# GEM3D/pressurePoissonSolver

Hardware: AMD Instinct MI355X
Metric: V-cycle lattice-site updates/sec, 512^3 3D Poisson (higher is better)
Workload: dtype f64; 1 GPU; apps/3d/steady-equivalent: 512^3 uniform, 4096 patches of 32^3, 5 levels, V(1,1), smoother=rbgs, Dirichlet, f ~ U(-1,1) splitmix64(0x5EED + patch id); workload_key=3d:u512:p32:rbgs, parallelism=patch-sharded x1 (Morton ranges), exchange=none, levels=5, smoother=rbgs

## Files before the change

### pressurepoissonsolver_amd/csrc/dispatch.hpp

```cpp
#pragma once
#include <cstddef>
#include <type_traits>

namespace tei
{
template <class F> inline auto dispatchN(int n, F f)
{
	switch (n) {
		case 4: return f(std::integral_constant<int, 4>{});
		case 8: return f(std::integral_constant<int, 8>{});
		case 16: return f(std::integral_constant<int, 16>{});
		default: return f(std::integral_constant<int, 32>{});
	}
}

template <class F> inline auto dispatchBool(bool b, F f)
{
	return b ? f(std::true_type{}) : f(std::false_type{});
}

template <int N, class F> inline void dispatchSlabs(int slabs, F f)
{
	switch (slabs) {
		case 1: f(std::integral_constant<int, 1>{}); break;
		case 2:
// ... 29 lines not shown
	}
	return zs;
}

inline int rbgsSlabCount(int n, int count, const SlabSwitches &s)
{
	if (s.pin) return pinnedSlabs(n, s.pin);
	int zs = 1;
	while (zs < 4 && !s.rbgs_noslab && (size_t) count * zs < 1024 && n / (zs * 2) >= 4) zs *= 2;
	if (zs == 4 && n == 32 && count <= 64 && !s.no_zs8) zs = 8;
	return zs;
}

constexpr size_t kResweepCacheBytes = (size_t) 160 << 20;

inline bool resweepPinValid(int pin) { return pin == 19 || pin == 27 || pin == 59; }

inline int resweepVariant(bool exported_terms, bool refined, int index, size_t level_bytes, int pin)
{
	if (exported_terms) return refined ? 0 : 3;
	const int v = pin ? pin : (index != 0 ? 27 : (level_bytes <= kResweepCacheBytes ? 19 : 59));
	return (refined && v == 19) ? 27 : v;
}
}
```

### pressurepoissonsolver_amd/csrc/gmg_core.hip

```cpp
#include "gmg_internal.hpp"

namespace tei
{
const char *kclassName[KC_COUNT] = {"stencil_apply", "stencil_resid", "stencil_jacobi", "stencil_rbgs",
                                    "cf_ghost", "restrict", "prolong_add", "patch_rhs", "dst_axis",
                                    "vecop", "reduce", "pack", "exchange", "stencil_rbgs_zero", "resid_restrict", "patch_solve_mfma", "stencil_rbgs_prolong",
                                    "stencil_rbgs_slabs", "stencil_slabs", "patch_solve_3pass", "rbgs_zero_resid_restrict",
                                    "restrict_fixup", "rbgs_resweep_prolong", "rbgs_zero_resid_restrict_faces",
                                    "rbgs_resweep_prolong_fcorr", "rbgs_zero_resid_restrict_faces_fcorr", "fcorr_gather", "patch_solve_mfma_faces",
                                    "bicg_update", "bicg_s", "bicg_p", "stencil_apply_dot", "patch_bcgs", "gradient", "divergence", "project", "prolong_linear", "prolong_quadratic", "boundary_restrict",
                                    "indicator", "regrid", "regrid_faces",
                                    "apply_coef", "resid_coef", "jacobi_coef", "rbgs_coef", "faces_restrict",
                                    "coef_split", "coef_merge",
                                    "faces_from_cells", "project_weighted", "boundary_rhs_w",
                                    "advect_flux", "advect", "faces_match", "faces_max_rate",
                                    "cell_slopes", "advect_flux_muscl", "advect_muscl"};
const char *optName[O_COUNT] = {"TE_2D_SIMPLE", "TE_2D_NO_MFMA", "TE_2D_NO_PF", "TE_2D_NO_MR_FUSE", "TE_2D_TPB", "TE_NO_FUSE2", "TE_NO_FUSE3",
                                "TE_NO_FUSE3_CF", "TE_NO_CFP", "TE_NO_XF", "TE_NO_FCORR", "TE_NO_FCORR_CF", "TE_NO_OVERLAP",
                                "TE_OVERLAP_MIN", "TE_NO_PS_FACES", "TE_PS_MODE", "TE_PS_SLOW", "TE_RBGS_NOSLAB", "TE_ZS_FORCE", "TE_NO_ZS8",
                                "TE_RESWEEP_V", "TE_EXCHANGE_TIMEOUT", "TE_NO_VERIFY", "TE_RCCL_LOOPBACK", "TE_NO_BICG_FUSE", "TE_POST_EXCHANGE", "TE_REPL_BLOCKS", "TE_PACK_FACES", "TE_OVERLAP_MODE", "TE_PUSH_TIMEOUT", "TE_NO_BICG_XF", "TE_PUSH_FAULT", "TE_2D_NO_FOLD", "TE_2D_NO_SYM", "TE_PUSH_NONFATAL", "TE_PS_NO_HALF", "TE_PS_HALF_MAX", "TE_NO_RS6_CF", "TE_NO_RS6_FIXUP", "TE_SCHUR_FULL", "TE_ZS_PIN"};

void drainEvents(te_gmg *g)
{
	if (g->ev_used == 0) return;
	(void) hipStreamSynchronize(g->stream);
	for (size_t i = 0; i < g->ev_used; i++) {
		float ms = 0;
		if (g->ev_pool[i].valid && hipEventElapsedTime(&ms, g->ev_pool[i].a, g->ev_pool[i].b) == hipSuccess) {
			g->calls[g->ev_pool[i].kc]++;
			g->total_ms[g->ev_pool[i].kc] += ms;
		}
	}
	g->ev_used = 0;
}

void Cfg::fromEnv()
{
	for (int o = 0; o < O_COUNT; o++) set(o, getenv(optName[o]));
}

static int parseSlabPin(const char *v)
{
	if (!v || !v[0] || v[1]) return 0;
// ... 25 lines not shown
	auto L = std::make_unique<LevelHost>();
	L->index = li;
	L->dim = T.dim, L->n = T.n, L->P = T.P, L->P_global = T.P_global, L->nc = T.nc, L->nf = T.nf;
	L->replicated = T.replicated, L->gathered = T.gathered;
	L->nif = T.nif, L->if_own = std::move(T.if_own), L->if_start = std::move(T.if_start), L->if_contrib = std::move(T.if_contrib);
	L->nbf = T.nbf, L->bface_host = std::move(T.bface), L->brestrict_host = std::move(T.brestrict);
	L->fx = std::move(T.fx), L->nremote = T.nremote;
	L->nslots = T.nslots, L->ncf = T.ncf, L->n_int = T.n_int, L->n_bnd = T.n_bnd;
	L->lds2d = T.lds2d, L->fuse2d = T.fuse2d, L->fuse2_ok = T.fuse2_ok;
	L->patch_vol = std::move(T.patch_vol);
	L->sym_ok = T.sym_ok, L->n_pure = T.n_pure, L->n_pure2 = T.n_pure2;
	L->Pc = T.Pc, L->n_up = T.n_up, L->n_down = T.n_down;
	L->tx_up = std::move(T.tx_up), L->tx_down = std::move(T.tx_down), L->tx_direct = std::move(T.tx_direct);
	L->prolong_fusable = T.prolong_fusable, L->prolong_fusable_cf = T.prolong_fusable_cf, L->has_copy = T.has_copy;
	L->repl_up = T.repl_up, L->repl_direct = T.repl_direct, L->post_exchange_free = T.post_exchange_free;
	L->tx_fup = std::move(T.tx_fup), L->up_foff_host = std::move(T.up_foff), L->down_foff_host = std::move(T.down_foff);
	L->up_ftotal = T.up_ftotal, L->down_ftotal = T.down_ftotal;

	const size_t P1 = (size_t) std::max(T.P, 1), nf = T.nf;
	const bool   fused3d = (D == 3 && T.fuse2_ok && T.P > 0);
	if ((rc = L->send_faces.upload(T.send_faces)) || (rc = L->sendbuf.alloc((size_t) std::max(T.nremote, 1) * nf))
	    || (rc = L->f6off.upload(T.f6off)) || (rc = L->order.upload(T.order)))
		return rc;
	if (D == 3 && ((rc = L->xfbuf[0].alloc(P1 * 2 * nf)) || (rc = L->xfbuf[1].alloc(P1 * 2 * nf)) || (rc = L->f6buf.alloc(P1 * 6 * nf))))
		return rc;
	if (fused3d && li > 0) {
		if ((rc = L->fcorr.alloc((size_t) T.P * 4 * nf))) return rc;
		HIPCHK(hipMemset(L->fcorr.p, 0, sizeof(double) * L->fcorr.n));
	}
	if (fused3d && (rc = L->rs6.alloc((size_t) T.P * 6 * nf / 4))) return rc;
	if ((rc = L->geom_starts.upload(T.geom_starts)) || (rc = L->geom_h.upload(T.geom_h)) || (rc = L->node_ids.upload(T.node_ids))
	    || (rc = L->cellvol.upload(T.cellvol)) || (rc = L->face_kind_patch.upload(T.face_kind_patch))
	    || (rc = L->face_kind.upload(T.face_kind)) || (rc = L->face_src.upload(T.face_src)) || (rc = L->face_kadj.upload(T.face_kadj))
	    || (rc = L->rh2.upload(T.rh2)) || (rc = L->cf_desc.upload(T.cf_desc)) || (rc = L->cf_slots.upload(T.cf_slots))
	    || (rc = L->ghost.alloc((size_t) std::max(T.nslots, 1) * nf)))
		return rc;
	if ((rc = L->matfrag.upload(T.matfrag)) || (rc = L->matsym.upload(T.matsym)) || (rc = L->matsT.upload(T.matsT))
	    || (rc = L->psinv.upload(T.psinv)) || (rc = L->psitab.upload(T.psitab)) || (rc = L->ps_list.upload(T.ps_list))
	    || (rc = L->mat2sym.upload(T.mat2sym)) || (rc = L->ps2_list.upload(T.ps2_list))
	    || (rc = L->corr.alloc(P1 * 2 * D * nf)) || (rc = L->plan.upload(T.plan)) || (rc = L->mats.upload(T.mats))
	    || (rc = L->lam.upload(T.lam)) || (rc = L->zero_mode.upload(T.zero_mode)))
		return rc;
	if (T.coarser
	    && ((D == 2 && T.fuse2_ok && (rc = L->e4buf.alloc(P1 * 4 * n))) || (rc = L->slot_parent.upload(T.slot_parent))
	        || (rc = L->slot_orth.upload(T.slot_orth)) || (rc = L->bc_desc.upload(T.bc_desc)) || (rc = L->cbase.upload(T.cbase))
	        || (rc = L->parent.upload(T.parent)) || (rc = L->orth.upload(T.orth)) || (rc = L->child.upload(T.child))
	        || (rc = L->copy.upload(T.copy)) || (rc = L->up_desc.upload(T.up_desc)) || (rc = L->down_desc.upload(T.down_desc))
	        || (rc = L->up_off.upload(T.up_off)) || (rc = L->down_off.upload(T.down_off))
	        || (rc = L->upbuf.alloc((size_t) std::max<int64_t>(T.up_total, 1)))
	        || (rc = L->downbuf.alloc((size_t) std::max<int64_t>(T.down_total, 1)))))
		return rc;
	g->levels.push_back(std::move(L));
	return TE_OK;
}

int newVec(te_gmg *g, int level, te_vec **out)
{
	LevelHost &L = *g->levels[level];
	auto       v = new te_vec;
	v->g         = g;
	v->level     = level;
	v->n         = (size_t) L.P * L.nc;
	hipError_t e = hipMalloc(&v->d, sizeof(double) * std::max<size_t>(v->n, 2));
	if (e != hipSuccess) {
		delete v;
		return te::fail(TE_EHIP, std::string("hipMalloc(vector): ") + hipGetErrorString(e));
	}
	e = hipMemsetAsync(v->d, 0, sizeof(double) * v->n, g->stream);
	if (e != hipSuccess) {
		(void) hipFree(v->d);
		delete v;
		return te::fail(TE_EHIP, std::string("hipMemsetAsync: ") + hipGetErrorString(e));
	}
	*out = v;
// ... 514 lines not shown
```

### pressurepoissonsolver_amd/csrc/gmg_fused3d.hip

```cpp
#include "gmg_ghosts3d.hpp"

namespace tei
{
template <int N>
int zeroSweepResidN(te_gmg *g, LevelHost &L, const double *f, double *out, double *coarse, double *xf_out, bool store_u,
                    double *fcorr_out, const double *fcorr_in, const PendingRhs *fs)
{
	RestrictDst rd = restrictDst(L, coarse);
	const bool export_rs6 = L.rs6.p && !store_u
	                        && (fcorr_out ? (L.prolong_fusable || !g->cfg.has(O_NO_RS6_CF))
	                                      : (L.Pc > 0 || L.n_up > 0) && !fcorr_in && !g->cfg.has(O_NO_RS6_FIXUP));
	rd.rs6                = export_rs6 ? L.rs6.p : nullptr;
	int rc;
	if (L.P > 0) {
		Timed      t(g, store_u ? KC_ZERO_RESID : (fcorr_in ? KC_ZERO_RESID_FACES_FCORR : KC_ZERO_RESID_FACES), (size_t) L.P * L.nc, true);
		if (!store_u) L.f6_tab = L.f6off.p != nullptr && !g->cfg.has(O_PACK_FACES);
		LevelDev   D = L.dev();
		const dim3 grid = slabGrid(L.P), blk(Tile3<N>::TPB);
		if (store_u) {
			D.xf_out = xf_out;
			launchT(t, (k_rbgs_zero_resid3d<N, true>), grid, blk, 0, g->stream, D, f, out, rd, FSrc());
		} else {
			D.f6_out = L.f6buf.p;
			D.fcorr  = fcorr_in;
// ... 19 lines not shown
			const int  key     = (export_rs6 ? 1 : 0) | (D.f6off ? 2 : 0);
			const bool rebuild = L.gdesc_key != key;
			if (rebuild) {
				int rc2 = L.gdesc.p ? TE_OK : L.gdesc.alloc((size_t) L.Pc * 48);
				if (rc2) return rc2;
				hipLaunchKernelGGL(k_gather_desc3d<N>, dim3(L.Pc), dim3(64), 0, g->stream, D, L.child.p, L.copy.p, export_rs6 ? 1 : 0, L.gdesc.p);
				L.gdesc_key = key;
			}
			if (rebuild || L.fcorr_zeroed_for != fcorr_out) {
				HIPCHK(hipMemsetAsync(fcorr_out, 0, sizeof(double) * (size_t) L.Pc * 4 * N * N, g->stream));
				L.fcorr_zeroed_for = fcorr_out;
			}
			Timed t(g, KC_FCORR_GATHER, (size_t) L.P * 6 * L.nf / 4);
			hipLaunchKernelGGL(k_fcorr_gather3d_v2<N>, dim3(L.Pc * 12), dim3(256), 0, g->stream, D, (const GatherDesc *) L.gdesc.p,
			                   export_rs6 ? (const double *) L.rs6.p : (const double *) nullptr, (const double *) L.f6buf.p, coarse, fcorr_out);
		}
	} else if (L.P > 0) {
		Timed    t(g, KC_FIXUP, (size_t) L.P * 6 * L.nf);
		LevelDev D = L.dev();
		if (store_u)
			D.xf = xf_out;
		else
			D.f6 = L.f6buf.p;
		hipLaunchKernelGGL((k_restrict_fixup3d<N, false>), dim3(L.P), dim3(256), 0, g->stream, D, out, rd);
	}
	if ((rc = shipRestricted<N>(g, L, coarse))) return rc;
	HIPCHK(hipGetLastError());
	return TE_OK;
}

template <int N>
int resweepProlongN(te_gmg *g, LevelHost &L, const double *f, double *out, const double *prolong_from, double *xf_out, const double *fcorr_in)
{
	ProlongSrc ps      = prolongSrc(L, prolong_from);
	const bool refined = L.ncf > 0 || L.has_copy;
	const int v = resweepVariant(fcorr_in != nullptr, refined, L.index, (size_t) L.P * L.nc * sizeof(double), g->resweep_pin);
	if (!v) return te::fail(TE_ESTATE, "resweepProlong: exported ghost terms on a refined level");
	auto launch = [&](LevelDev D) {
		if (D.count == 0) return;
		Timed t(g, fcorr_in ? KC_RESWEEP_FCORR : KC_RESWEEP, (size_t) D.count * L.nc, true);
		D.f6    = L.f6buf.p;
		D.fcorr = fcorr_in;
		const dim3 grid = slabGrid(D.count), blk(Tile3<N>::TPB);
		if (refined) {
			if (v == 59)
				launchT(t, (k_rbgs_resweep_prolong3d<N, 59, false, true>), grid, blk, 0, g->stream, D, f, out, ps);
			else
				launchT(t, (k_rbgs_resweep_prolong3d<N, 27, false, true>), grid, blk, 0, g->stream, D, f, out, ps);
		} else if (v == 3) {
			launchT(t, (k_rbgs_resweep_prolong3d<N, 3, true>), grid, blk, 0, g->stream, D, f, out, ps);
		} else if (v == 19) {
			launchT(t, (k_rbgs_resweep_prolong3d<N, 19>), grid, blk, 0, g->stream, D, f, out, ps);
		} else if (v == 59) {
			launchT(t, (k_rbgs_resweep_prolong3d<N, 59>), grid, blk, 0, g->stream, D, f, out, ps);
		} else {
			launchT(t, (k_rbgs_resweep_prolong3d<N, 27>), grid, blk, 0, g->stream, D, f, out, ps);
		}
	};
	if (L.post_exchange_free && L.ghost_has_v && !refined && !g->cfg.has(O_POST_EXCHANGE)) {
		ps.gparent    = L.slot_parent.p;
		ps.gorth      = L.slot_orth.p;
		L.ghost_has_v = false;
		LevelDev D    = L.dev();
		D.xf_out      = xf_out;
		launch(D);
		HIPCHK(hipGetLastError());
		return TE_OK;
	}
	int rc = withGhosts<N>(g, L, {nullptr, L.f6buf.p, &ps}, launch, nullptr, xf_out);
	if (rc) return rc;
	HIPCHK(hipGetLastError());
	return TE_OK;
}
// ... 50 lines not shown
```

### pressurepoissonsolver_amd/csrc/gmg_ghosts3d.hpp

```cpp
#pragma once
#include "dispatch.hpp"
#include "gmg_internal.hpp"

namespace tei
{
struct GhostSrc {
	const double     *u;
	const double     *f6 = nullptr;
	const ProlongSrc *ps = nullptr;
};

template <int N> bool packFaces(te_gmg *g, LevelHost &L, const GhostSrc &src, bool may_push = false)
{
	const bool push = may_push && g->push.on && L.push_faces && !g->recording && L.push_face_dst[0].p;
	Timed      t(g, push ? KC_EXCHANGE : KC_PACK, (size_t) L.nremote * L.nf);
	const dim3 grid(L.nremote), blk(N * N < 256 ? N * N : 256);
	PackPush   pp;
	if (push) {
		pushBegin(g, L, 1);
		pp.dst    = L.push_face_dst[L.push_par].p;
		pp.flags  = L.push_face_flags.p;
		pp.nflags = (int) L.push_face_flags.n;
		pp.epoch  = L.push_ep;
		pp.raise  = pushRaiseValue(g, L.push_ep);
// ... 72 lines not shown
		launch(L.devPart(true));
		HIPCHK(hipStreamWaitEvent(g->stream, g->ev_recv, 0));
		return TE_OK;
	}
	packFaces<N>(g, L, src);
	HIPCHK(hipEventRecord(g->ev_pack, g->stream));
	HIPCHK(hipStreamWaitEvent(g->comm_stream, g->ev_pack, 0));
	int rc = faceExchange(g, L, L.sendbuf.p, g->comm_stream);
	if (rc) return rc;
	HIPCHK(hipEventRecord(g->ev_recv, g->comm_stream));
	launch(L.devPart(false));
	HIPCHK(hipStreamWaitEvent(g->stream, g->ev_recv, 0));
	if (L.ncf > 0) cfGhosts<N>(g, L, src);
	launch(L.devPart(true));
	return TE_OK;
}

template <int N> inline int stencilSlabs(const te_gmg *g, int P) { return stencilSlabCount(N, P, slabSwitches(g)); }

template <int N> inline int rbgsSlabs(const te_gmg *g, int count) { return rbgsSlabCount(N, count, slabSwitches(g)); }

inline dim3 slabGrid(int count, int zs = 1) { return dim3(8 * ((count * zs + 7) / 8)); }

inline RestrictDst restrictDst(const LevelHost &L, double *coarse)
{
	RestrictDst rd = RestrictDst();
	rd.parent     = L.parent.p;
	rd.orth       = L.orth.p;
	rd.coarse     = coarse;
	rd.remote     = L.upbuf.p;
	rd.remote_off = L.up_off.p;
	return rd;
}

inline ProlongSrc prolongSrc(const LevelHost &L, const double *coarse)
{
	ProlongSrc ps;
	ps.parent = L.parent.p;
	ps.orth   = L.orth.p;
	ps.coarse = coarse;
	return ps;
}

template <int N> int shipRestricted(te_gmg *g, LevelHost &L, double *coarse)
{
	if (L.repl_up && L.repl_direct && !g->cfg.has(O_REPL_BLOCKS)) {
// ... 18 lines not shown
```

### pressurepoissonsolver_amd/csrc/gmg_internal.hpp

```cpp
#pragma once
#include "capi_common.hpp"
#include "dispatch.hpp"
#include "level_tables.hpp"
#include <hip/hip_ext.h>
#include <rccl/rccl.h>
#include "kernels3d.hpp"
#include "march3d.hpp"
#include "kernels2d.hpp"
#include "patchsolve32.hpp"
#include "patchsolve32_sym.hpp"
#include "patchsolve16.hpp"
#include "initkernels.hpp"
#include "bckernels.hpp"
#include "pushkernels.hpp"
#include <algorithm>
#include <array>
#include <atomic>
#include <chrono>
#include <cmath>
#include <cstdio>
#include <cstring>
#include <dlfcn.h>
#include <map>
#include <memory>
// ... 32 lines not shown
	KC_APPLY, KC_RESID, KC_JACOBI, KC_RBGS, KC_CFGHOST, KC_RESTRICT, KC_PROLONG, KC_PATCH_RHS,
	KC_DST, KC_VECOP, KC_REDUCE, KC_PACK, KC_EXCHANGE, KC_RBGS_ZERO, KC_RESID_RESTRICT, KC_PS_MFMA, KC_RBGS_PROLONG,
	KC_RBGS_SLABS, KC_STENCIL_SLABS, KC_PS_3PASS, KC_ZERO_RESID, KC_FIXUP, KC_RESWEEP, KC_ZERO_RESID_FACES,
	KC_RESWEEP_FCORR, KC_ZERO_RESID_FACES_FCORR, KC_FCORR_GATHER,
	KC_PS_MFMA_FACES,
	KC_BICG_UPDATE, KC_BICG_S, KC_BICG_P, KC_APPLY_DOT,
	KC_PATCH_BCGS,
	KC_GRADIENT, KC_DIVERGENCE, KC_PROJECT,
	KC_PROLONG_LINEAR,
	KC_PROLONG_QUADRATIC, KC_BOUNDARY_RESTRICT,
	KC_INDICATOR, KC_REGRID,
	KC_FACE_REGRID,
	KC_APPLY_COEF, KC_RESID_COEF, KC_JACOBI_COEF, KC_RBGS_COEF, KC_FACES_RESTRICT,
	KC_COEF_SPLIT, KC_COEF_MERGE,
	KC_FACES_FROM_CELLS, KC_PROJECT_WEIGHTED, KC_BOUNDARY_RHS_W,
	KC_ADVECT_FLUX, KC_ADVECT, KC_FACES_MATCH, KC_FACES_RATE,
	KC_CELL_SLOPES, KC_ADVECT_FLUX_MUSCL, KC_ADVECT_MUSCL, KC_COUNT
};
extern const char *kclassName[KC_COUNT];

enum Opt : int {
	O_2D_SIMPLE, O_2D_NO_MFMA, O_2D_NO_PF, O_2D_NO_MR_FUSE, O_2D_TPB, O_NO_FUSE2, O_NO_FUSE3, O_NO_FUSE3_CF, O_NO_CFP, O_NO_XF,
	O_NO_FCORR, O_NO_FCORR_CF, O_NO_OVERLAP, O_OVERLAP_MIN, O_NO_PS_FACES, O_PS_MODE, O_PS_SLOW, O_RBGS_NOSLAB,
	O_ZS_FORCE, O_NO_ZS8, O_RESWEEP_V, O_EXCHANGE_TIMEOUT, O_NO_VERIFY, O_RCCL_LOOPBACK, O_NO_BICG_FUSE, O_POST_EXCHANGE, O_REPL_BLOCKS, O_PACK_FACES, O_OVERLAP_MODE, O_PUSH_TIMEOUT, O_NO_BICG_XF, O_PUSH_FAULT, O_2D_NO_FOLD, O_2D_NO_SYM, O_PUSH_NONFATAL, O_PS_NO_HALF, O_PS_HALF_MAX, O_NO_RS6_CF, O_NO_RS6_FIXUP, O_SCHUR_FULL, O_ZS_PIN, O_COUNT
};
extern const char *optName[O_COUNT];
inline bool optStructural(int o) { return o == O_2D_SIMPLE || o == O_NO_CFP || o == O_2D_NO_MR_FUSE || o == O_NO_OVERLAP || o == O_EXCHANGE_TIMEOUT; }
struct Cfg {
	bool        on[O_COUNT] = {};
	std::string val[O_COUNT];
	void        set(int o, const char *v)
	{
		on[o]  = v != nullptr;
		val[o] = v ? v : "";
	}
	void fromEnv();
	bool        has(int o) const { return on[o]; }
	const char *str(int o) const { return on[o] ? val[o].c_str() : nullptr; }
	int         num(int o, int dflt) const { return on[o] ? atoi(val[o].c_str()) : dflt; }
	double      real(int o, double dflt) const { return on[o] ? atof(val[o].c_str()) : dflt; }
};

struct SetupAcc {
	double malloc_ms = 0, copy_ms = 0, nmalloc = 0;
};
inline thread_local SetupAcc *g_setup_acc = nullptr;
struct SetupClock {
// ... 162 lines not shown
	std::vector<double *> push_peer_cf[2];
	DevBuf<unsigned>      push_done;
	DevBuf<double *>             push_face_dst[2];
	DevBuf<PushFlag>             push_face_flags;
	int                push_par = 0;
	unsigned long long push_ep  = 0;
	PushWait           push_wait;
	bool   repl_direct = false;
	ExPlan tx_direct;
	DevBuf<double> fcorr;
	bool           f_has_corr = false;
	Fold2DHost     fold_pending;
	DevBuf<double> rs6;
	DevBuf<GatherDesc> gdesc;
	int                gdesc_key = -1;
	const double      *fcorr_zeroed_for = nullptr;
	DevBuf<double> e4buf;
	bool ps_faces = false;
	DevBuf<double> xfbuf[2];
	int            xf_cur       = 0;
	const double  *xf_valid_for = nullptr;
	DevBuf<int32_t> order;
	int             n_int = 0, n_bnd = 0;
	int             overlap_mode = -1;
	LevelDev        devPart(bool boundary) const
	{
		LevelDev L = dev();
		L.order    = order.p;
		L.first    = boundary ? n_int : 0;
		L.count    = boundary ? n_bnd : n_int;
		return L;
	}
};

struct PendingRhs {
	int    kind;
	FSrc   args;
	size_t n2;
};
struct EventPair {
	hipEvent_t a, b;
	int        kc;
	bool       valid;
};
}
using namespace tei;
// ... 454 lines not shown
```

### pressurepoissonsolver_amd/csrc/gmg_launch3d.hip

```cpp
#include "gmg_ghosts3d.hpp"

namespace tei
{
template <int N, int MODE, int ZS>
void launchStencilZS(te_gmg *g, dim3 grid, const LevelDev &D_, const double *u, const double *f, double *out, double omega,
                     const RestrictDst &rd, int redmode, const RedSrc &rs)
{
	const dim3 blk(Tile3<N>::TPB);
	const LevelDev &D = stamped(g, D_, MODE == MODE_RESID_RESTRICT ? "stencil resid+restrict" : "stencil", grid.x);
	if constexpr (MODE == MODE_APPLY) {
		if (redmode == RED_OUT_A) {
			hipLaunchKernelGGL((k_stencil3d<N, MODE, ZS, RED_OUT_A>), grid, blk, 0, g->stream, D, u, f, out, omega, rd, rs);
			return;
		}
		if (redmode == RED_OUT_A_OUT) {
			hipLaunchKernelGGL((k_stencil3d<N, MODE, ZS, RED_OUT_A_OUT>), grid, blk, 0, g->stream, D, u, f, out, omega, rd, rs);
			return;
		}
	}
	if constexpr (MODE == MODE_RESID) {
		if (redmode == RED_OUT_OUT) {
			hipLaunchKernelGGL((k_stencil3d<N, MODE, ZS, RED_OUT_OUT>), grid, blk, 0, g->stream, D, u, f, out, omega, rd, rs);
			return;
		}
// ... 44 lines not shown
}

template <int N, bool ZERO, bool PROLONG>
void launchRbgsKernel(te_gmg *g, const LevelDev &D_, const double *u, const double *f, double *out, const ProlongSrc &ps)
{
	const int  zs = rbgsSlabs<N>(g, D_.count);
	const dim3 grid = slabGrid(D_.count, zs), blk(Tile3<N>::TPB);
	const LevelDev &D = stamped(g, D_, ZERO ? "rbgs from zero" : (PROLONG ? "rbgs on u + P e" : "rbgs"), grid.x);
	dispatchSlabs<N>(zs, [&](auto z) {
		hipLaunchKernelGGL((k_rbgs3d<N, ZERO, PROLONG, decltype(z)::value>), grid, blk, 0, g->stream, D, u, f, out, ps);
	});
}

template <int N> int launchRbgsN(te_gmg *g, LevelHost &L, const double *u, const double *f, double *out, bool zero_guess,
                                 const double *prolong_from, const double *xf_in, double *xf_out)
{
	if (prolong_from) {
		ProlongSrc ps = prolongSrc(L, prolong_from);
		ps.cbase      = L.cbase.p;
		const bool cfp = (L.ncf > 0 || L.has_copy);
		if (!cfp && !ps.cbase) return te::fail(TE_ESTATE, "launchRbgs: fused prolongation on a level without its coarse-base table");
		auto launch = [&](LevelDev D) {
			if (D.count == 0) return;
			if (cfp) {
				Timed t(g, KC_RBGS_PROLONG, (size_t) D.count * L.nc);
				hipLaunchKernelGGL((k_rbgs3d<N, false, true, 1, true>), slabGrid(D.count), dim3(Tile3<N>::TPB), 0, g->stream, D, u, f, out, ps);
				return;
			}
			Timed t(g, rbgsSlabs<N>(g, D.count) > 1 ? KC_RBGS_SLABS : KC_RBGS_PROLONG, (size_t) D.count * L.nc);
			launchRbgsKernel<N, false, true>(g, D, u, f, out, ps);
		};
		int rc = withGhosts<N>(g, L, {u, nullptr, &ps}, launch, xf_in, xf_out);
		if (rc) return rc;
		HIPCHK(hipGetLastError());
		return TE_OK;
	}
	if (zero_guess) {
		Timed    t(g, rbgsSlabs<N>(g, L.P) > 1 ? KC_RBGS_SLABS : KC_RBGS_ZERO, (size_t) L.P * L.nc);
		LevelDev D = L.dev();
		D.xf_out   = xf_out;
		launchRbgsKernel<N, true, false>(g, D, u, f, out, ProlongSrc());
		HIPCHK(hipGetLastError());
		return TE_OK;
	}
	auto launch = [&](LevelDev D) {
		if (D.count == 0) return;
// ... 87 lines not shown
```

### pressurepoissonsolver_amd/csrc/level_tables.cpp

```cpp
#include "level_tables.hpp"
#include "capi_common.hpp"
#include "table_layout.hpp"
#include <algorithm>
#include <array>
#include <cmath>
#include <map>
#include <tuple>

using namespace te;

namespace tei
{
namespace
{
using PeerItems = std::vector<std::pair<int, int64_t>>;

void transformMatrix(int type, int n, double *m)
{
	static const double oi[6] = {0.0, 0.5, 0.5, 1.0, 0.5, 0.5}, oj[6] = {0.5, 0.0, 0.5, 0.5, 1.0, 0.5};
	for (int i = 0; i < n; i++) {
		for (int j = 0; j < n; j++) {
			const double x = M_PI / n * ((i + oi[type]) * (j + oj[type]));
			m[i * n + j]   = type < 3 ? cos(x) : sin(x);
		}
// ... 195 lines not shown
					int nb = (q < NQ) ? lv.g_nbr[gf * 4 + q] : -1;
					if (nb >= 0 && lv.g_rank[nb] != me)
						cfd.push_back(-(remote_slot.at(std::make_tuple(p, s, q)) + 2));
					else
						cfd.push_back(nb >= 0 ? lv.g_local[nb] : -1);
				}
				T.cf_slots.push_back(T.nslots);
				T.nslots++;
			}
			ghost |= (fk[p * NS + s] == FACE_GHOST);
		}
		(ghost ? bnd : T.order).push_back(p);
		auto it = plan_of_key.find(key);
		if (it == plan_of_key.end()) {
			it = plan_of_key.emplace(key, (int) keys.size()).first;
			keys.push_back(key);
		}
		T.plan[p] = it->second;
	}
	T.ncf   = (int) T.cf_slots.size();
	T.n_int = (int) T.order.size();
	T.n_bnd = (int) bnd.size();
	T.order.insert(T.order.end(), bnd.begin(), bnd.end());
	T.face_kind_patch = fk;
	for (auto &k : T.face_kind_patch)
		if (k >= FACE_LOCAL) k = FACE_DIRICHLET;
	return keys;
}

void planTransforms(const std::vector<int> &keys, int D, int n, LevelTables &T)
{
	const int np = (int) keys.size(), NS = 2 * D;
	T.mats.assign((size_t) np * 2 * D * n * n, 0.0);
	T.lam.assign((size_t) np * D * n, 0.0);
	T.zero_mode.assign(np, 0);
	for (int k = 0; k < np; k++) {
		const int key  = keys[k];
		T.zero_mode[k] = (key == (1 << NS) - 1);
		for (int a = 0; a < D; a++) {
			static const int    fwd[4] = {3, 2, 5, 0}, inv[4] = {4, 2, 5, 1};
			static const double shift[4] = {1.0, 0.5, 0.5, 0.0};
			const int           ends = (key >> (2 * a)) & 3;
			transformMatrix(fwd[ends], n, &T.mats[((size_t) k * 2 * D + a) * n * n]);
			transformMatrix(inv[ends], n, &T.mats[((size_t) k * 2 * D + D + a) * n * n]);
			for (int i = 0; i < n; i++) {
				const double s = sin((i + shift[ends]) * M_PI / (2 * n));
// ... 247 lines not shown
		std::sort(bc.begin(), bc.end());
		T.up_total  = layOut(bc, T.up_total, T.up_desc, T.up_off, none);
		T.up_ftotal = layOutFaces(bc, T.up_ftotal, D, n, T.up_foff, fnone);
		for (auto &b : bc) {
			T.bc_desc.push_back(parent[b.patch]);
			T.bc_desc.push_back(b.o);
		}
	}
	T.down_total  = layOut(down, 0, T.down_desc, T.down_off, downs);
	T.down_ftotal = layOutFaces(down, 0, D, n, T.down_foff, fdowns);
	for (size_t i = 0; i < down.size(); i++)
		child[(size_t) down[i].patch * NCH + std::max(down[i].o, 0)] = -((int) i + 2);
	for (int pc = 0; pc < cv.P; pc++) {
		if (copy[pc]) continue;
		for (int o = 0; o < NCH; o++)
			if (child[(size_t) pc * NCH + o] == -1) return te::fail(TE_EINVAL, "te_gmg_create: coarse patch with a missing child");
	}
	T.Pc     = cv.P;
	T.n_up   = (int) (T.up_desc.size() / 2);
	T.n_down = (int) down.size();
	const bool parents_local = up.empty() && (down.empty() || T.repl_up);
	const bool all_children  = std::all_of(orth.begin(), orth.end(), [](int32_t o) { return o >= 0; });
	T.has_copy               = !all_children;
	T.prolong_fusable        = (D == 3 && T.ncf == 0 && parents_local && all_children);
	T.prolong_fusable_cf     = (D == 3 && parents_local && !opt.no_cfp);
	if (D == 2 && T.lds2d && parents_local) {
		T.fuse2d          = true;
		T.prolong_fusable = ((opt.no_mr_fuse_2d ? T.nslots == 0 : T.ncf == 0) && all_children);
	}
	if (D == 2 && T.lds2d) T.fuse2_ok = uniformlyRefined(lv);
	if (T.repl_up) {
		replicatedPlans(H, lv, cv, recvs, downs, T);
		T.tx_fup = replicatedUpPlan(H, fdowns, T.up_ftotal);
	} else {
		T.tx_up   = mergePlan(ups, downs);
		T.tx_down = mergePlan(downs, ups);
		T.tx_fup  = mergePlan(fups, fdowns);
	}
	if (T.prolong_fusable && D == 3) {
		const int64_t nn = (int64_t) n * n, nnn = nn * n, hh = n / 2;
		auto          base = [&](int p) {
            const int o = orth[p];
            return (int64_t) parent[p] * nnn + ((o & 1) ? hh : 0) + n * ((o & 2) ? hh : 0) + nn * ((o & 4) ? hh : 0);
		};
		T.cbase.assign((size_t) std::max(P, 1) * 7, -1);
		for (int p = 0; p < P; p++) {
// ... 74 lines not shown
```

### pressurepoissonsolver_amd/csrc/level_tables.hpp

```cpp
#pragma once
#include "mesh.hpp"
#include <cstddef>
#include <cstdint>
#include <vector>

namespace tei
{
struct ExPlan {
	std::vector<int32_t> peers;
	std::vector<int64_t> send_off, send_cnt, recv_off, recv_cnt;
	bool empty() const { return peers.empty(); }
};

struct LevelBuildOpts {
	bool simple_2d = false, no_cfp = false, no_mr_fuse_2d = false;
};

struct LevelTables {
	int    dim = 3, n = 0, P = 0, P_global = 0;
	bool   replicated = false, gathered = false;
	size_t nc = 0, nf = 0;
	ExPlan               fx;
	int                  nremote = 0;
	std::vector<int32_t> send_faces, f6off;
	std::vector<int32_t> face_kind, face_kind_patch, face_src, cf_desc, cf_slots, order, node_ids;
	std::vector<double>  face_kadj, rh2, cellvol, patch_vol, geom_starts, geom_h;
	int                  nslots = 0, ncf = 0, n_int = 0, n_bnd = 0;
	bool                 lds2d = false, fuse2d = false, fuse2_ok = false;
	std::vector<int32_t> plan, zero_mode, psitab, ps_list, ps2_list;
	std::vector<double>  mats, lam, matsT, matfrag, matsym, psinv, mat2sym;
	bool                 sym_ok = false;
	int                  n_pure = 0, n_pure2 = 0;
	bool                 coarser = false;
	int                  Pc = 0, n_up = 0, n_down = 0;
	std::vector<int32_t> parent, orth, child, copy, up_desc, down_desc, bc_desc, slot_parent, slot_orth;
	std::vector<int64_t> up_off, down_off, cbase;
	int64_t              up_total = 0, down_total = 0;
	ExPlan               tx_up, tx_down, tx_direct;
	std::vector<int64_t> up_foff, down_foff;
	int64_t              up_ftotal = 0, down_ftotal = 0;
	ExPlan               tx_fup;
	bool prolong_fusable = false, prolong_fusable_cf = false, has_copy = false, repl_up = false, repl_direct = false,
	     post_exchange_free = false;
	int                  nif = -1;
	std::vector<int32_t> if_own, if_start, if_contrib;
	int                  nbf = 0;
	std::vector<int32_t> bface;
	std::vector<int32_t> brestrict;
};

inline int64_t faceDoubles(int dim, int64_t m) { return dim == 3 ? 3 * m * m * m + 3 * m * m : 2 * m * m + 2 * m; }

int computeLevelTables(const te::Hierarchy &H, int li, const LevelBuildOpts &o, LevelTables &out);

}
```

### pressurepoissonsolver_amd/csrc/march3d.hpp

```cpp
#pragma once
#include "kernels3d.hpp"
#include <type_traits>

namespace te
{
template <bool NT> __device__ __forceinline__ double2 ldStream(const double2 *p)
{
	if (NT) {
		double2 v;
		v.x = __builtin_nontemporal_load(&p->x);
		v.y = __builtin_nontemporal_load(&p->y);
		return v;
	}
	return *p;
}
template <bool NT> __device__ __forceinline__ void stStream(double2 *p, double2 v)
{
	if (NT) {
		__builtin_nontemporal_store(v.x, &p->x);
		__builtin_nontemporal_store(v.y, &p->y);
	} else
		*p = v;
}
__device__ __forceinline__ double2 takeRegs(const double2 &src)
// ... 1234 lines not shown
							g = L.f6[f6Face<N>(L.f6off, src, s ^ 1) + a + N * b];
						else if (ax == 0 && L.xf)
							g = L.xf[((size_t) src * 2 + ((s & 1) ^ 1)) * NN + a + N * b];
						else
							g = u[(size_t) src * NNN + oth + a * sa + b * sb];
						if (OWN) {
							if (L.f6)
								g += L.f6[f6Face<N>(L.f6off, p, s) + a + N * b];
							else if (ax == 0 && L.xf)
								g += L.xf[((size_t) p * 2 + (s & 1)) * NN + a + N * b];
							else
								g += u[(size_t) p * NNN + ((s & 1) ? (N - 1) * sn : 0) + a * sa + b * sb];
						}
						acc += (w * g) / 8;
					}
				const int ca = (ax == 0) ? 1 : 0, cbx = (ax == 2) ? 1 : 2;
				cb[ha * cs[ca] + hb * cs[cbx] + ((s & 1) ? (H - 1) * cs[ax] : 0)] += acc;
			}
		}
		__syncthreads();
	}
}

template <int N>
__global__ void k_pack_faces6_3d(const int32_t *__restrict__ faces, const double *__restrict__ f6, ProlongSrc ps,
                                 double *__restrict__ sendbuf, const int32_t *__restrict__ f6off, PackPush pp = PackPush())
{
	constexpr int NN = N * N, H = N / 2;
	const int     p = faces[2 * blockIdx.x], s = faces[2 * blockIdx.x + 1];
	const int     ax = s >> 1;
	const int     sa = (ax == 0) ? N : 1, sb = (ax == 2) ? N : NN, sn = (ax == 0) ? 1 : (ax == 1 ? N : NN);
	const double *fp = f6 + f6Face<N>(f6off, p, s);
	double       *o  = pp.dst ? pp.dst[blockIdx.x] : sendbuf + (size_t) blockIdx.x * NN;
	if (pp.dst && *pp.err) {
	} else if (ps.coarse && ps.orth[p] < 0) {
		const int face = (s & 1) ? (N - 1) * sn : 0;
		for (int i = threadIdx.x; i < NN; i += blockDim.x) o[i] = fp[i] + coarseAtCell<N>(ps, p, face + (i % N) * sa + (i / N) * sb);
	} else {
		const double *cp = ps.coarse ? coarseOctant<N>(ps, p) + ((s & 1) ? (H - 1) * sn : 0) : nullptr;
		for (int i = threadIdx.x; i < NN; i += blockDim.x) {
			const int a = i % N, b = i / N;
			o[i] = cp ? fp[i] + cp[(a / 2) * sa + (b / 2) * sb] : fp[i];
		}
	}
	packPushTail(pp);
}
// ... 353 lines not shown
```

Baseline: 149.3 billion lattice-site updates/s.

## Add one-pass restrict fixup kernel and optional reversed post-smooth patch order

```diff
diff --git a/pressurepoissonsolver_amd/csrc/dispatch.hpp b/pressurepoissonsolver_amd/csrc/dispatch.hpp
--- a/pressurepoissonsolver_amd/csrc/dispatch.hpp
+++ b/pressurepoissonsolver_amd/csrc/dispatch.hpp
@@ -1,6 +1,8 @@
 #pragma once
 #include <cstddef>
+#include <cstdint>
 #include <type_traits>
+#include <vector>
 
 namespace tei
 {
@@ -76,4 +78,21 @@
 	const int v = pin ? pin : (index != 0 ? 27 : (level_bytes <= kResweepCacheBytes ? 19 : 59));
 	return (refined && v == 19) ? 27 : v;
 }
+
+constexpr size_t kReverseMinBytes = (size_t) 32 << 20;
+
+inline bool reversePost(int nranks, size_t level_bytes, bool on, bool off, bool pin)
+{
+	if (off || nranks != 1) return false;
+	return pin || (on && level_bytes > kReverseMinBytes && level_bytes <= kResweepCacheBytes);
 }
+
+inline std::vector<int32_t> reversedOrder(int P)
+{
+	std::vector<int32_t> o((size_t) (P > 0 ? P : 0));
+	for (int i = 0; i < P; i++) o[(size_t) i] = P - 1 - i;
+	return o;
+}
+
+inline bool fixupOnePass(bool own, bool octants_local, bool off) { return !own && octants_local && !off; }
+}
diff --git a/pressurepoissonsolver_amd/csrc/gmg_core.hip b/pressurepoissonsolver_amd/csrc/gmg_core.hip
--- a/pressurepoissonsolver_amd/csrc/gmg_core.hip
+++ b/pressurepoissonsolver_amd/csrc/gmg_core.hip
@@ -18,7 +18,8 @@
 const char *optName[O_COUNT] = {"TE_2D_SIMPLE", "TE_2D_NO_MFMA", "TE_2D_NO_PF", "TE_2D_NO_MR_FUSE", "TE_2D_TPB", "TE_NO_FUSE2", "TE_NO_FUSE3",
                                 "TE_NO_FUSE3_CF", "TE_NO_CFP", "TE_NO_XF", "TE_NO_FCORR", "TE_NO_FCORR_CF", "TE_NO_OVERLAP",
                                 "TE_OVERLAP_MIN", "TE_NO_PS_FACES", "TE_PS_MODE", "TE_PS_SLOW", "TE_RBGS_NOSLAB", "TE_ZS_FORCE", "TE_NO_ZS8",
-                                "TE_RESWEEP_V", "TE_EXCHANGE_TIMEOUT", "TE_NO_VERIFY", "TE_RCCL_LOOPBACK", "TE_NO_BICG_FUSE", "TE_POST_EXCHANGE", "TE_REPL_BLOCKS", "TE_PACK_FACES", "TE_OVERLAP_MODE", "TE_PUSH_TIMEOUT", "TE_NO_BICG_XF", "TE_PUSH_FAULT", "TE_2D_NO_FOLD", "TE_2D_NO_SYM", "TE_PUSH_NONFATAL", "TE_PS_NO_HALF", "TE_PS_HALF_MAX", "TE_NO_RS6_CF", "TE_NO_RS6_FIXUP", "TE_SCHUR_FULL", "TE_ZS_PIN"};
+                                "TE_RESWEEP_V", "TE_EXCHANGE_TIMEOUT", "TE_NO_VERIFY", "TE_RCCL_LOOPBACK", "TE_NO_BICG_FUSE", "TE_POST_EXCHANGE", "TE_REPL_BLOCKS", "TE_PACK_FACES", "TE_OVERLAP_MODE", "TE_PUSH_TIMEOUT", "TE_NO_BICG_XF", "TE_PUSH_FAULT", "TE_2D_NO_FOLD", "TE_2D_NO_SYM", "TE_PUSH_NONFATAL", "TE_PS_NO_HALF", "TE_PS_HALF_MAX", "TE_NO_RS6_CF", "TE_NO_RS6_FIXUP", "TE_SCHUR_FULL", "TE_ZS_PIN",
+                                "TE_REVERSE_POST", "TE_NO_REVERSE_POST", "TE_REVERSE_POST_PIN", "TE_NO_FIXUP_V2", "TE_RESWEEP_FCORR_NT"};
 
 void drainEvents(te_gmg *g)
 {
@@ -90,6 +91,7 @@
 	if ((rc = L->send_faces.upload(T.send_faces)) || (rc = L->sendbuf.alloc((size_t) std::max(T.nremote, 1) * nf))
 	    || (rc = L->f6off.upload(T.f6off)) || (rc = L->order.upload(T.order)))
 		return rc;
+	L->octants_local = T.octants_local;
 	if (D == 3 && ((rc = L->xfbuf[0].alloc(P1 * 2 * nf)) || (rc = L->xfbuf[1].alloc(P1 * 2 * nf)) || (rc = L->f6buf.alloc(P1 * 6 * nf))))
 		return rc;
 	if (fused3d && li > 0) {
@@ -118,6 +120,7 @@
 	        || (rc = L->upbuf.alloc((size_t) std::max<int64_t>(T.up_total, 1)))
 	        || (rc = L->downbuf.alloc((size_t) std::max<int64_t>(T.down_total, 1)))))
 		return rc;
+	if (D == 3 && (rc = L->order_rev.upload(T.order_rev))) return rc;
 	g->levels.push_back(std::move(L));
 	return TE_OK;
 }
diff --git a/pressurepoissonsolver_amd/csrc/gmg_fused3d.hip b/pressurepoissonsolver_amd/csrc/gmg_fused3d.hip
--- a/pressurepoissonsolver_amd/csrc/gmg_fused3d.hip
+++ b/pressurepoissonsolver_amd/csrc/gmg_fused3d.hip
@@ -65,12 +65,17 @@
 			D.xf = xf_out;
 		else
 			D.f6 = L.f6buf.p;
-		hipLaunchKernelGGL((k_restrict_fixup3d<N, false>), dim3(L.P), dim3(256), 0, g->stream, D, out, rd);
+		if (fixupOnePass(false, L.octants_local, g->cfg.has(O_NO_FIXUP_V2)))
+			hipLaunchKernelGGL(k_restrict_fixup3d_v2<N>, dim3(L.P), dim3(256), 0, g->stream, D, out, rd);
+		else
+			hipLaunchKernelGGL((k_restrict_fixup3d<N, false>), dim3(L.P), dim3(256), 0, g->stream, D, out, rd);
 	}
 	if ((rc = shipRestricted<N>(g, L, coarse))) return rc;
 	HIPCHK(hipGetLastError());
 	return TE_OK;
 }
+
+static bool resweepFcorrNt(const te_gmg *g) { return g->cfg.has(O_RESWEEP_FCORR_NT); }
 
 template <int N>
 int resweepProlongN(te_gmg *g, LevelHost &L, const double *f, double *out, const double *prolong_from, double *xf_out, const double *fcorr_in)
@@ -84,6 +89,7 @@
 		Timed t(g, fcorr_in ? KC_RESWEEP_FCORR : KC_RESWEEP, (size_t) D.count * L.nc, true);
 		D.f6    = L.f6buf.p;
 		D.fcorr = fcorr_in;
+		postOrder(g, L, D);
 		const dim3 grid = slabGrid(D.count), blk(Tile3<N>::TPB);
 		if (refined) {
 			if (v == 59)
@@ -91,7 +97,12 @@
 			else
 				launchT(t, (k_rbgs_resweep_prolong3d<N, 27, false, true>), grid, blk, 0, g->stream, D, f, out, ps);
 		} else if (v == 3) {
-			launchT(t, (k_rbgs_resweep_prolong3d<N, 3, true>), grid, blk, 0, g->stream, D, f, out, ps);
+			bool nt = false;
+			if constexpr (N == 32) {
+				nt = resweepFcorrNt(g);
+				if (nt) launchT(t, (k_rbgs_resweep_prolong3d<N, 19, true>), grid, blk, 0, g->stream, D, f, out, ps);
+			}
+			if (!nt) launchT(t, (k_rbgs_resweep_prolong3d<N, 3, true>), grid, blk, 0, g->stream, D, f, out, ps);
 		} else if (v == 19) {
 			launchT(t, (k_rbgs_resweep_prolong3d<N, 19>), grid, blk, 0, g->stream, D, f, out, ps);
 		} else if (v == 59) {
diff --git a/pressurepoissonsolver_amd/csrc/gmg_ghosts3d.hpp b/pressurepoissonsolver_amd/csrc/gmg_ghosts3d.hpp
--- a/pressurepoissonsolver_amd/csrc/gmg_ghosts3d.hpp
+++ b/pressurepoissonsolver_amd/csrc/gmg_ghosts3d.hpp
@@ -118,6 +118,14 @@
 
 inline dim3 slabGrid(int count, int zs = 1) { return dim3(8 * ((count * zs + 7) / 8)); }
 
+inline void postOrder(const te_gmg *g, const LevelHost &L, LevelDev &D)
+{
+	if (D.order || D.first != 0 || D.count != L.P || !L.order_rev.p) return;
+	if (reversePost(g->nranks, (size_t) L.P * L.nc * sizeof(double), g->cfg.has(O_REVERSE_POST), g->cfg.has(O_NO_REVERSE_POST),
+	                g->cfg.has(O_REVERSE_POST_PIN)))
+		D.order = L.order_rev.p;
+}
+
 inline RestrictDst restrictDst(const LevelHost &L, double *coarse)
 {
 	RestrictDst rd = RestrictDst();
diff --git a/pressurepoissonsolver_amd/csrc/gmg_internal.hpp b/pressurepoissonsolver_amd/csrc/gmg_internal.hpp
--- a/pressurepoissonsolver_amd/csrc/gmg_internal.hpp
+++ b/pressurepoissonsolver_amd/csrc/gmg_internal.hpp
@@ -78,7 +78,8 @@
 enum Opt : int {
 	O_2D_SIMPLE, O_2D_NO_MFMA, O_2D_NO_PF, O_2D_NO_MR_FUSE, O_2D_TPB, O_NO_FUSE2, O_NO_FUSE3, O_NO_FUSE3_CF, O_NO_CFP, O_NO_XF,
 	O_NO_FCORR, O_NO_FCORR_CF, O_NO_OVERLAP, O_OVERLAP_MIN, O_NO_PS_FACES, O_PS_MODE, O_PS_SLOW, O_RBGS_NOSLAB,
-	O_ZS_FORCE, O_NO_ZS8, O_RESWEEP_V, O_EXCHANGE_TIMEOUT, O_NO_VERIFY, O_RCCL_LOOPBACK, O_NO_BICG_FUSE, O_POST_EXCHANGE, O_REPL_BLOCKS, O_PACK_FACES, O_OVERLAP_MODE, O_PUSH_TIMEOUT, O_NO_BICG_XF, O_PUSH_FAULT, O_2D_NO_FOLD, O_2D_NO_SYM, O_PUSH_NONFATAL, O_PS_NO_HALF, O_PS_HALF_MAX, O_NO_RS6_CF, O_NO_RS6_FIXUP, O_SCHUR_FULL, O_ZS_PIN, O_COUNT
+	O_ZS_FORCE, O_NO_ZS8, O_RESWEEP_V, O_EXCHANGE_TIMEOUT, O_NO_VERIFY, O_RCCL_LOOPBACK, O_NO_BICG_FUSE, O_POST_EXCHANGE, O_REPL_BLOCKS, O_PACK_FACES, O_OVERLAP_MODE, O_PUSH_TIMEOUT, O_NO_BICG_XF, O_PUSH_FAULT, O_2D_NO_FOLD, O_2D_NO_SYM, O_PUSH_NONFATAL, O_PS_NO_HALF, O_PS_HALF_MAX, O_NO_RS6_CF, O_NO_RS6_FIXUP, O_SCHUR_FULL, O_ZS_PIN,
+	O_REVERSE_POST, O_NO_REVERSE_POST, O_REVERSE_POST_PIN, O_NO_FIXUP_V2, O_RESWEEP_FCORR_NT, O_COUNT
 };
 extern const char *optName[O_COUNT];
 inline bool optStructural(int o) { return o == O_2D_SIMPLE || o == O_NO_CFP || o == O_2D_NO_MR_FUSE || o == O_NO_OVERLAP || o == O_EXCHANGE_TIMEOUT; }
@@ -287,6 +288,8 @@
 	const double  *xf_valid_for = nullptr;
 	DevBuf<int32_t> order;
 	int             n_int = 0, n_bnd = 0;
+	DevBuf<int32_t> order_rev;
+	bool            octants_local = false;
 	int             overlap_mode = -1;
 	LevelDev        devPart(bool boundary) const
 	{
diff --git a/pressurepoissonsolver_amd/csrc/gmg_launch3d.hip b/pressurepoissonsolver_amd/csrc/gmg_launch3d.hip
--- a/pressurepoissonsolver_amd/csrc/gmg_launch3d.hip
+++ b/pressurepoissonsolver_amd/csrc/gmg_launch3d.hip
@@ -90,6 +90,7 @@
 		if (!cfp && !ps.cbase) return te::fail(TE_ESTATE, "launchRbgs: fused prolongation on a level without its coarse-base table");
 		auto launch = [&](LevelDev D) {
 			if (D.count == 0) return;
+			postOrder(g, L, D);
 			if (cfp) {
 				Timed t(g, KC_RBGS_PROLONG, (size_t) D.count * L.nc);
 				hipLaunchKernelGGL((k_rbgs3d<N, false, true, 1, true>), slabGrid(D.count), dim3(Tile3<N>::TPB), 0, g->stream, D, u, f, out, ps);
diff --git a/pressurepoissonsolver_amd/csrc/level_tables.cpp b/pressurepoissonsolver_amd/csrc/level_tables.cpp
--- a/pressurepoissonsolver_amd/csrc/level_tables.cpp
+++ b/pressurepoissonsolver_amd/csrc/level_tables.cpp
@@ -1,5 +1,6 @@
 #include "level_tables.hpp"
 #include "capi_common.hpp"
+#include "dispatch.hpp"
 #include "table_layout.hpp"
 #include <algorithm>
 #include <array>
@@ -241,6 +242,7 @@
 	T.n_int = (int) T.order.size();
 	T.n_bnd = (int) bnd.size();
 	T.order.insert(T.order.end(), bnd.begin(), bnd.end());
+	T.order_rev = reversedOrder(P);
 	T.face_kind_patch = fk;
 	for (auto &k : T.face_kind_patch)
 		if (k >= FACE_LOCAL) k = FACE_DIRICHLET;
@@ -534,6 +536,7 @@
 	const bool parents_local = up.empty() && (down.empty() || T.repl_up);
 	const bool all_children  = std::all_of(orth.begin(), orth.end(), [](int32_t o) { return o >= 0; });
 	T.has_copy               = !all_children;
+	T.octants_local          = up.empty() && all_children;
 	T.prolong_fusable        = (D == 3 && T.ncf == 0 && parents_local && all_children);
 	T.prolong_fusable_cf     = (D == 3 && parents_local && !opt.no_cfp);
 	if (D == 2 && T.lds2d && parents_local) {
diff --git a/pressurepoissonsolver_amd/csrc/level_tables.hpp b/pressurepoissonsolver_amd/csrc/level_tables.hpp
--- a/pressurepoissonsolver_amd/csrc/level_tables.hpp
+++ b/pressurepoissonsolver_amd/csrc/level_tables.hpp
@@ -23,7 +23,7 @@
 	ExPlan               fx;
 	int                  nremote = 0;
 	std::vector<int32_t> send_faces, f6off;
-	std::vector<int32_t> face_kind, face_kind_patch, face_src, cf_desc, cf_slots, order, node_ids;
+	std::vector<int32_t> face_kind, face_kind_patch, face_src, cf_desc, cf_slots, order, order_rev, node_ids;
 	std::vector<double>  face_kadj, rh2, cellvol, patch_vol, geom_starts, geom_h;
 	int                  nslots = 0, ncf = 0, n_int = 0, n_bnd = 0;
 	bool                 lds2d = false, fuse2d = false, fuse2_ok = false;
@@ -42,6 +42,7 @@
 	ExPlan               tx_fup;
 	bool prolong_fusable = false, prolong_fusable_cf = false, has_copy = false, repl_up = false, repl_direct = false,
 	     post_exchange_free = false;
+	bool octants_local = false;
 	int                  nif = -1;
 	std::vector<int32_t> if_own, if_start, if_contrib;
 	int                  nbf = 0;
diff --git a/pressurepoissonsolver_amd/csrc/march3d.hpp b/pressurepoissonsolver_amd/csrc/march3d.hpp
--- a/pressurepoissonsolver_amd/csrc/march3d.hpp
+++ b/pressurepoissonsolver_amd/csrc/march3d.hpp
@@ -1280,6 +1280,153 @@
 	}
 }
 
+struct FixFace {
+	const double *p;
+	int           s1a, s1b, sda, sdb;
+	int           mode;
+};
+template <int N>
+__device__ __forceinline__ FixFace fixFace(const LevelDev &L, const double *__restrict__ u, const RestrictDst &rd, int p, int s, int kind,
+                                           int src, int fo, const double *dummy)
+{
+	constexpr int NN = N * N, NNN = N * N * N, H = N / 2;
+	const int     ax = s >> 1;
+	const bool    local = kind == FACE_LOCAL, ghost = kind == FACE_GHOST;
+	const int     sl = local ? src : p;
+	const bool    fin = rd.rs6 && local, x_cols = ax == 0 && L.xf;
+	const bool    compact = ghost || L.f6 || x_cols;
+	const int     sn = (ax == 0) ? 1 : (ax == 1 ? N : NN);
+	const int     sa = compact ? 1 : ((ax == 0) ? N : 1), sb = compact ? N : ((ax == 2) ? N : NN);
+	const double *pr = rd.rs6 + ((size_t) sl * 6 + (s ^ 1)) * (H * H);
+	const double *pg = L.ghost + (size_t) (ghost ? src : 0) * NN;
+	const double *p6 = L.f6 + (size_t) fo * NN;
+	const double *px = L.xf + ((size_t) sl * 2 + ((s & 1) ^ 1)) * NN;
+	const double *pu = u + (size_t) sl * NNN + ((s & 1) ? 0 : (N - 1) * sn);
+	FixFace       f;
+	f.mode = !(local || ghost) ? 0 : (fin ? 1 : 2);
+	f.p    = f.mode == 0 ? dummy : (fin ? pr : (ghost ? pg : (L.f6 ? p6 : (x_cols ? px : pu))));
+	f.s1a  = f.mode == 0 ? 0 : (fin ? 1 : 2 * sa);
+	f.s1b  = f.mode == 0 ? 0 : (fin ? H : 2 * sb);
+	f.sda  = f.mode == 2 ? sa : 0;
+	f.sdb  = f.mode == 2 ? sb : 0;
+	return f;
+}
+__device__ __forceinline__ int fixLoad(const FixFace &lo, const FixFace &hi, bool on, bool high, int ha, int hb, const double *dummy,
+                                       double (&g)[4])
+{
+	const FixFace &F = high ? hi : lo;
+	const double  *q = on ? F.p + (ha * F.s1a + hb * F.s1b) : dummy;
+	const int      da = on ? F.sda : 0, db = on ? F.sdb : 0;
+	g[0] = q[0], g[1] = q[da], g[2] = q[db], g[3] = q[da + db];
+	return on ? F.mode : 0;
+}
+__device__ __forceinline__ double fixTerm(int mode, double w, const double (&g)[4])
+{
+#pragma clang fp contract(off)
+	double acc = 0.0;
+	acc += (w * g[0]) / 8;
+	acc += (w * g[1]) / 8;
+	acc += (w * g[2]) / 8;
+	acc += (w * g[3]) / 8;
+	return mode == 1 ? g[0] : acc;
+}
+template <int N>
+__global__ __launch_bounds__(256) void k_restrict_fixup3d_v2(LevelDev L, const double *__restrict__ u, RestrictDst rd)
+{
+	constexpr int NN = N * N, NNN = N * N * N, H = N / 2, HI = H > 2 ? H - 2 : 1;
+	constexpr int NZ = 2 * H * H, NY = 2 * H * (H - 2), NX = 2 * (H - 2) * (H - 2);
+	constexpr int KZ = (NZ + 255) / 256, KY = (NY + 255) / 256, KX = (NX + 255) / 256;
+	const int     p = L.first + blockIdx.x, tid = threadIdx.x;
+	const int     pa_ = rd.parent[p], o_ = rd.orth[p];
+	int           kind[6], src[6], fo[6];
+#pragma unroll
+	for (int s = 0; s < 6; s++) kind[s] = L.face_kind[(size_t) p * 6 + s], src[s] = L.face_src[(size_t) p * 6 + s];
+	const double *dummy = L.rh2 + (size_t) p * 3;
+	const double  wx = -dummy[0], wy = -dummy[1], wz = -dummy[2];
+	const int32_t *tab = L.f6off ? L.f6off : L.face_src;
+#pragma unroll
+	for (int s = 0; s < 6; s++) {
+		const int at = (kind[s] == FACE_LOCAL ? src[s] : p) * 6 + (s ^ 1), e = tab[at];
+		fo[s]        = L.f6off ? e : at;
+	}
+	const bool    ok = pa_ >= 0 && o_ >= 0;
+	const int     pa = ok ? pa_ : 0, o = ok ? o_ : 0;
+	double       *cb = rd.coarse + (size_t) pa * NNN + ((o & 1) ? H : 0) + N * ((o & 2) ? H : 0) + NN * ((o & 4) ? H : 0);
+	const FixFace W = fixFace<N>(L, u, rd, p, 0, kind[0], src[0], fo[0], dummy), E = fixFace<N>(L, u, rd, p, 1, kind[1], src[1], fo[1], dummy),
+	              S = fixFace<N>(L, u, rd, p, 2, kind[2], src[2], fo[2], dummy), Nf = fixFace<N>(L, u, rd, p, 3, kind[3], src[3], fo[3], dummy),
+	              B = fixFace<N>(L, u, rd, p, 4, kind[4], src[4], fo[4], dummy), T = fixFace<N>(L, u, rd, p, 5, kind[5], src[5], fo[5], dummy);
+	auto cellZ = [&](int k, int &cx, int &cy, int &cz) {
+		const int i = tid + 256 * k, ic = i < NZ ? i : 0, r = ic % (H * H);
+		cx = r % H, cy = r / H, cz = (ic / (H * H)) * (H - 1);
+		return ok && i < NZ;
+	};
+	auto cellY = [&](int k, int &cx, int &cy, int &cz) {
+		const int i = tid + 256 * k, ic = i < NY ? i : 0, r = ic % (H * HI);
+		cx = r % H, cz = 1 + r / H, cy = (ic / (H * HI)) * (H - 1);
+		return ok && i < NY;
+	};
+	auto cellX = [&](int k, int &cx, int &cy, int &cz) {
+		const int i = tid + 256 * k, ic = i < NX ? i : 0, r = ic % (HI * HI);
+		cy = 1 + r % HI, cz = 1 + r / HI, cx = (ic / (HI * HI)) * (H - 1);
+		return ok && i < NX;
+	};
+	auto edge = [](int c) { return c == 0 || c == H - 1; };
+	double fz[KZ], gz[KZ][3][4], fy[KY ? KY : 1], gy[KY ? KY : 1][2][4], fx[KX ? KX : 1], gx[KX ? KX : 1][4];
+	int    mz[KZ][3], my[KY ? KY : 1][2], mx[KX ? KX : 1];
+#pragma unroll
+	for (int k = 0; k < KZ; k++) {
+		int cx, cy, cz;
+		cellZ(k, cx, cy, cz);
+		mz[k][0] = fixLoad(S, Nf, edge(cy), cy == H - 1, cx, cz, dummy, gz[k][0]);
+		mz[k][1] = fixLoad(B, T, true, cz == H - 1, cx, cy, dummy, gz[k][1]);
+		mz[k][2] = fixLoad(W, E, edge(cx), cx == H - 1, cy, cz, dummy, gz[k][2]);
+		fz[k]    = cb[cx + N * cy + NN * cz];
+	}
+#pragma unroll
+	for (int k = 0; k < KY; k++) {
+		int cx, cy, cz;
+		cellY(k, cx, cy, cz);
+		my[k][0] = fixLoad(S, Nf, true, cy == H - 1, cx, cz, dummy, gy[k][0]);
+		my[k][1] = fixLoad(W, E, edge(cx), cx == H - 1, cy, cz, dummy, gy[k][1]);
+		fy[k]    = cb[cx + N * cy + NN * cz];
+	}
+#pragma unroll
+	for (int k = 0; k < KX; k++) {
+		int cx, cy, cz;
+		cellX(k, cx, cy, cz);
+		mx[k] = fixLoad(W, E, true, cx == H - 1, cy, cz, dummy, gx[k]);
+		fx[k] = cb[cx + N * cy + NN * cz];
+	}
+	{
+#pragma clang fp contract(off)
+#pragma unroll
+		for (int k = 0; k < KZ; k++) {
+			int        cx, cy, cz;
+			const bool valid = cellZ(k, cx, cy, cz);
+			double     f     = fz[k];
+			if (mz[k][0]) f = f + fixTerm(mz[k][0], wy, gz[k][0]);
+			if (mz[k][1]) f = f + fixTerm(mz[k][1], wz, gz[k][1]);
+			if (mz[k][2]) f = f + fixTerm(mz[k][2], wx, gz[k][2]);
+			if (valid && (mz[k][0] | mz[k][1] | mz[k][2])) cb[cx + N * cy + NN * cz] = f;
+		}
+#pragma unroll
+		for (int k = 0; k < KY; k++) {
+			int        cx, cy, cz;
+			const bool valid = cellY(k, cx, cy, cz);
+			double     f     = fy[k];
+			if (my[k][0]) f = f + fixTerm(my[k][0], wy, gy[k][0]);
+			if (my[k][1]) f = f + fixTerm(my[k][1], wx, gy[k][1]);
+			if (valid && (my[k][0] | my[k][1])) cb[cx + N * cy + NN * cz] = f;
+		}
+#pragma unroll
+		for (int k = 0; k < KX; k++) {
+			int        cx, cy, cz;
+			const bool valid = cellX(k, cx, cy, cz);
+			if (valid && mx[k]) cb[cx + N * cy + NN * cz] = fx[k] + fixTerm(mx[k], wx, gx[k]);
+		}
+	}
+}
+
 template <int N>
 __global__ void k_pack_faces6_3d(const int32_t *__restrict__ faces, const double *__restrict__ f6, ProlongSrc ps,
                                  double *__restrict__ sendbuf, const int32_t *__restrict__ f6off, PackPush pp = PackPush())
```

Result: no change. 149.1 billion lattice-site updates/s (-0.1%).
